# osmosis-diffusion/osmosis-diffusion-code

Hardware: AMD Instinct MI355X
Metric: denoise-steps/sec (256x256 RGBD, 1000-step DDPM+guidance) (higher is better)
Workload: dtype f32 (f16x3 conv)

## Files before the change

osmosis_diffusion_code_amd/_lib.py:

```python
import ctypes as C
import os
import threading
from typing import List, Optional, Tuple

import torch

_HERE = os.path.dirname(os.path.abspath(__file__))
LIB_PATH = os.environ.get("OSM_LIB") or os.path.join(_HERE, "libosmosis_hip.so")

c_float_p = C.c_void_p


class OsmosisHipError(RuntimeError):
    pass


class ConvDesc(C.Structure):
    _fields_ = [("x", C.c_void_p), ("w", C.c_void_p), ("bias", C.c_void_p), ("res", C.c_void_p),
                ("y", C.c_void_p), ("splitk_ws", C.c_void_p),
                ("B", C.c_int), ("H", C.c_int), ("W", C.c_int), ("Cin", C.c_int), ("Cout", C.c_int),
                ("ksize", C.c_int), ("splitk", C.c_int), ("accumulate", C.c_int),
                ("ldx", C.c_longlong), ("ldy", C.c_longlong), ("ldr", C.c_longlong), ("wfmt", C.c_int),
                ("gn_table", C.c_void_p), ("gn_silu", C.c_int),
                ("colsum", C.c_void_p), ("stat_mode", C.c_int), ("stat_silu", C.c_int), ("stat_x", C.c_void_p),
# ... 183 lines not shown
                                _P, _P, _I, _I, _P, _P],
}
EXPORTS_PHYSGROUP = sorted(_SIGS_PHYSGROUP)
_D = C.c_double
_SIGS_BLIND = {
    "osm_psf_tap_grad": [_P, _P, _P, _P, _I, _I, _I, _I, _I, _LL, _LL, _I, _I, _P, _P],
    "osm_psf_tap_step": [_P, _P, _P, _I, _I, _I, _LL, _D, _D, _P],
    "osm_ps_blind_optimize": [_P, _P, _P, _P, _P, _P, _I, _I, _I, _I, _I, _I, _I, _P, _P, _P, _P, _P, _P, _I, _D, _D, _P],
}
EXPORTS_BLIND = sorted(_SIGS_BLIND)
_SIGS_DEPTHPRIOR = {
    "osm_depth_nblk": [_I],
    "osm_depth_reduce": [C.POINTER(DepthDesc), _P, _P, _P, _P, _P],
    "osm_depth_fit": [C.POINTER(DepthDesc), _P, _P, _P, _P],
    "osm_depth_grad": [C.POINTER(DepthDesc), _P, _P, _P, _P, _P, _P],
    "osm_depth_loss_grad": [C.POINTER(DepthDesc), _P, _P, _P, _P, _P, _P, _P, _P],
}
EXPORTS_DEPTHPRIOR = sorted(_SIGS_DEPTHPRIOR)
_SIGS_SOLVER = {
    "osm_solver_update_c": [_P, _P, _P, _P, _P, _P, _P, _P, _P, _F, _P, _P, _P, _I, _I, _I, _P],
    "osm_solver_update_rng_c": [_P, _P, _P, _P, _P, _P, _P, _P, _F, _P, _P, _P, _I, _I, _I, C.c_ulonglong, _P, _I, _I, _I, _I, _P],
}
EXPORTS_SOLVER = sorted(_SIGS_SOLVER)

_lib = None
_lock = threading.Lock()


def load():
    global _lib
    if _lib is not None:
        return _lib
    with _lock:
        if _lib is None:
            if not os.path.exists(LIB_PATH):
                raise OsmosisHipError(
                    f"{LIB_PATH} is missing: build it with `python -c 'import __graft_entry__ as g; g.build()'` "
                    "or `make -C osmosis_diffusion_code_amd/csrc` (hipcc, --offload-arch=gfx950). "
                    "There is no CPU fallback for the product path.")
            lib = C.CDLL(LIB_PATH)
            for name, argtypes in list(_SIGS.items()) + list(_SIGS_LINOP.items()) + list(_SIGS_PSF.items()) + list(_SIGS_PHYSLIN.items()) + \
                    list(_SIGS_PHYSGROUP.items()) + list(_SIGS_BLIND.items()) + list(_SIGS_DEPTHPRIOR.items()) + list(_SIGS_SOLVER.items()):
                fn = getattr(lib, name)
                fn.argtypes = argtypes
                fn.restype = C.c_int
            lib.osm_packed_weight_elems.argtypes = [_I, _I, _I, _I, _I]
            lib.osm_packed_weight_elems.restype = C.c_longlong
            lib.osm_winograd_weight_elems.argtypes = [_I, _I, _I, _I]
            lib.osm_winograd_weight_elems.restype = C.c_longlong
            lib.osm_quantile_abs_ws_bytes.argtypes = [_LL]
            lib.osm_quantile_abs_ws_bytes.restype = C.c_longlong
            lib.osm_last_error.argtypes = []
            lib.osm_last_error.restype = C.c_char_p
            _lib = lib
    return _lib


class Recorder:

    def __init__(self):
        self.calls: List[Tuple] = []
        self.keep: List = []

    def __enter__(self):
        _state.recorders.append(self)
        return self

    def __exit__(self, *exc):
        _state.recorders.pop()
        return False

    @staticmethod
    def suspended():
        class _Suspend:
# ... 99 lines not shown
```

osmosis_diffusion_code_amd/csrc/guidance.hip:

```cpp
#include "osm_common.h"
#include "depth_conv.h"
#include "../../include/osmosis_linop.h"
#include "../../include/osmosis_psf.h"
#include "../../include/osmosis_physlin.h"
#include "../../include/osmosis_physgroup.h"
#include "../../include/osmosis_solver.h"

namespace {

constexpr int PPB = 1024;
constexpr int NRED = 16;

template <bool MASKED> struct PixMask { float wm[3]; };
template <> struct PixMask<false> {};

template <bool MASKED>
struct Pix : PixMask<MASKED> {
  float rgb[3], D, y[3];
  float d, dd, w;
  float Ea[3], Eb[3], J[3], r[3];
};

template <bool MASKED, bool FMA_I = false, bool MODEL_ONLY = false>
__device__ __forceinline__ void eval_pixel(const osm_phys_desc& ds, const float* __restrict__ x0,
                                           const float* __restrict__ y, const float* __restrict__ mask,
                                           const float* __restrict__ phi, int b, int p, Pix<MASKED>& q) {
  const long long base = (long long)b * 4 * ds.HW + p;
  float m[3] = {1.f, 1.f, 1.f};
#pragma unroll
  for (int c = 0; c < 3; ++c) {
    q.rgb[c] = x0[base + (long long)c * ds.HW];
    if constexpr (!MODEL_ONLY) q.y[c] = y[(long long)b * 3 * ds.HW + (long long)c * ds.HW + p];
    if constexpr (MASKED) m[c] = mask[(long long)b * 3 * ds.HW + (long long)c * ds.HW + p];
  }
  q.D = x0[base + 3LL * ds.HW];
  if (ds.kind == 3) {
    q.d = 0.f; q.dd = 0.f; q.w = 1.f;
#pragma unroll
    for (int c = 0; c < 3; ++c) {
      q.Ea[c] = q.Eb[c] = 1.f;
      q.J[c] = 0.5f * (q.rgb[c] + 1.0f);
      q.r[c] = q.y[c] - q.rgb[c];
      if constexpr (MASKED) { q.wm[c] = m[c]; q.r[c] *= m[c]; }
    }
    return;
  }
  q.d = conv_depth(q.D, ds.depth_type, ds.dval, q.dd);
  float wdd;
  q.w = ds.weight_type == 1 ? conv_depth(q.D, ds.wdepth_type, ds.wval, wdd) : 1.0f;
  const float* ph = phi + b * 9;
#pragma unroll
  for (int c = 0; c < 3; ++c) {
    const float pa = ds.kind == 2 ? ph[0] : ph[c];
    const float pb = ds.kind == 0 ? ph[3 + c] : pa;
    const float pinf = ph[6 + c];
    q.Ea[c] = expf(-pa * q.d);
    q.Eb[c] = expf(-pb * q.d);
    q.J[c] = 0.5f * (q.rgb[c] + 1.0f);
    float I;
    if constexpr (FMA_I) {
      I = fmaf(q.J[c], q.Ea[c], pinf * (1.0f - q.Eb[c]));
    } else {
      I = q.J[c] * q.Ea[c] + pinf * (1.0f - q.Eb[c]);
    }
    if constexpr (MODEL_ONLY) {
      q.r[c] = I;
    } else if constexpr (MASKED) {
      q.wm[c] = q.w * m[c];
      q.r[c] = (q.y[c] - (2.0f * I - 1.0f)) * q.wm[c];
    } else {
      q.r[c] = (q.y[c] - (2.0f * I - 1.0f)) * q.w;
    }
  }
}

template <bool MASKED, bool LIN>
__global__ __launch_bounds__(256) void phys_reduce_kernel(osm_phys_desc ds, const float* __restrict__ x0,
                                                           const float* __restrict__ y,
                                                           const float* __restrict__ mask,
                                                           const float* __restrict__ phi, const float* __restrict__ v,
                                                           float* __restrict__ part, int nblk) {
  static_assert(!(MASKED && LIN), "the composed route's mask acts on the measurement's grid (phys_resid_kernel)");
  __shared__ float red[4][NRED];
  const int b = blockIdx.y, blk = blockIdx.x;
  float s[NRED];
#pragma unroll
  for (int k = 0; k < NRED; ++k) s[k] = 0.f;
  const int pend = min(ds.HW, (blk + 1) * PPB);
  const float* ph = phi + b * 9;
  for (int p = blk * PPB + threadIdx.x; p < pend; p += 256) {
    Pix<MASKED> q;
    eval_pixel<MASKED, false, LIN>(ds, x0, y, mask, phi, b, p, q);
#pragma unroll
    for (int c = 0; c < 3; ++c) {
      const float pinf = ph[6 + c];
      float k2;
      if constexpr (LIN) {
        k2 = v[((long long)b * 3 + c) * ds.HW + p];
      } else {
        float wc = q.w;
        if constexpr (MASKED) wc = q.wm[c];
        k2 = -2.0f * wc * q.r[c];
        s[0] += q.r[c] * q.r[c];
      }
      s[1 + c] += k2 * (-q.d * q.J[c] * q.Ea[c]);
      s[4 + c] += k2 * (pinf * q.d * q.Eb[c]);
      s[7 + c] += k2 * (1.0f - q.Eb[c]);
      s[10 + c] += q.rgb[c];
      const float e = fmaxf(fabsf(q.rgb[c]) - 0.7f, 0.0f);
      s[13] += e * e;
    }
  }
  const int lane = threadIdx.x & 63, wv = threadIdx.x >> 6;
#pragma unroll
  for (int k = 0; k < NRED; ++k) {
    const float t = osm::wave_sum(s[k]);
    if (lane == 0) red[wv][k] = t;
  }
  __syncthreads();
  if (threadIdx.x < NRED) {
    const int k = threadIdx.x;
    part[((long long)b * nblk + blk) * NRED + k] = (red[0][k] + red[1][k]) + (red[2][k] + red[3][k]);
  }
}

__device__ __forceinline__ float sgn(float v) { return (v > 0.f) ? 1.f : ((v < 0.f) ? -1.f : 0.f); }

__device__ __forceinline__ int phys_param_lr(const osm_phys_desc& ds, float* lr) {
  for (int i = 0; i < 9; ++i) lr[i] = 0.f;
  int live;
  if (ds.kind == 0) {
    for (int c = 0; c < 3; ++c) { lr[c] = ds.eta[0]; lr[3 + c] = ds.eta[1]; }
    live = 0x3f;
  } else if (ds.kind == 1) {
    for (int c = 0; c < 3; ++c) lr[c] = ds.eta[0];
    live = 0x7;
  } else {
    lr[0] = ds.eta[0];
    live = 0x1;
  }
  for (int c = 0; c < 3; ++c) lr[6 + c] = ds.eta[2];
  return live | 0x1c0;
}

__device__ __forceinline__ void phys_param_grad(const osm_phys_desc& ds, const double* tot, double gscale, double* dg) {
  for (int i = 0; i < 9; ++i) dg[i] = 0.0;
  if (ds.kind == 0) {
    for (int c = 0; c < 3; ++c) {
// ... 93 lines not shown
}

template <bool LIN> struct FinLin { const float* part_r; int nblk_r, hw; };
template <> struct FinLin<false> {};

template <bool LIN>
__device__ __forceinline__ void fin_walk(const float* __restrict__ part, float* __restrict__ red, int nblk, const FinLin<LIN>& lin,
                                         int b, int lane, double* tot) {
  static_assert(NRED * 4 == 64, "one wave covers the components");
  const int comp = lane >> 2, sub = lane & 3;
  double a = 0.0;
#pragma unroll 4
  for (int k = sub; k < nblk; k += 4) a += (double)part[((long long)b * nblk + k) * NRED + comp];
  if constexpr (LIN) {
    if (comp == 0) {
      a = 0.0;
      for (int k = sub; k < lin.nblk_r; k += 4) a += (double)lin.part_r[(long long)b * lin.nblk_r + k];
    }
  }
  a += __shfl_xor(a, 1, 64);
  a += __shfl_xor(a, 2, 64);
  if (sub == 0) {
    tot[comp] = a;
    red[b * NRED + comp] = (float)a;
  }
}

template <bool LIN>
__device__ __forceinline__ bool fin_member(const osm_phys_desc& ds, const double* tot, const FinLin<LIN>& lin, int zero_guard, int b,
                                           float* __restrict__ loss_out, int do_update, double* dg) {
  double n = 3.0 * (double)ds.HW;
  if constexpr (LIN) n = 3.0 * (double)lin.hw;
  double L, gscale;
  bool live = true;
  if (ds.loss_type == 0) {
    L = sqrt(tot[0]);
    gscale = 1.0 / L;
    if (zero_guard && tot[0] == 0.0) { gscale = 0.0; live = false; }
  } else {
    L = tot[0] / n;
    gscale = 2.0 / n;
  }
  if (loss_out) loss_out[b] = (float)L;
  if (do_update) phys_param_grad(ds, tot, gscale, dg);
  return live;
}

__device__ __forceinline__ void fin_step(const osm_phys_desc& ds, const double* dg, double omega, float* ph, float* st) {
  float g[9], lr[9];
  const int live = phys_param_lr(ds, lr);
  for (int i = 0; i < 9; ++i) g[i] = (float)(dg[i] * omega);
  phys_opt_step(ds, g, lr, live, ph, st);
}

template <bool LIN>
__global__ void phys_finalize_kernel(osm_phys_desc ds, const float* __restrict__ part, float* __restrict__ red,
                                     float* __restrict__ phi, int do_update, float* __restrict__ loss_out,
                                     float* __restrict__ opt_state, int nblk, int zero_guard, const FinLin<LIN> lin) {
  __shared__ double tot[NRED];
  const int b = blockIdx.x;
  fin_walk(part, red, nblk, lin, b, threadIdx.x, tot);
  __syncthreads();
  if (threadIdx.x == 0) {
    double dg[9];
    if (fin_member(ds, tot, lin, zero_guard, b, loss_out, do_update, dg) && do_update)
      fin_step(ds, dg, 1.0, phi + b * 9, opt_state ? opt_state + b * 20 : nullptr);
  }
}

struct GroupOff { int G, reduce_mean, off[OSM_MAX_GROUPS + 1]; };
constexpr int GWAVES = 4;

template <bool LIN>
__global__ __launch_bounds__(64 * GWAVES) void phys_finalize_group_kernel(osm_phys_desc ds, const float* __restrict__ part,
                                                                          float* __restrict__ red, float* phi, int do_update,
                                                                          float* __restrict__ loss_out, float* opt_state, int nblk,
                                                                          int zero_guard, const GroupOff go, const FinLin<LIN> lin) {
  __shared__ double tot[GWAVES][NRED];
  __shared__ double dsh[GWAVES][9];
  __shared__ int live_sh[GWAVES];
  __shared__ float row[9 + 20];
  __shared__ int stepped;
  const int b0 = go.off[blockIdx.x], n = go.off[blockIdx.x + 1] - b0;
  const int wv = threadIdx.x >> 6, lane = threadIdx.x & 63;
  double acc[9];
  int any = 0;
  for (int r0 = 0; r0 < n; r0 += GWAVES) {
    const int m = r0 + wv;
    if (m < n) fin_walk(part, red, nblk, lin, b0 + m, lane, tot[wv]);
    __syncthreads();
// ... 9 lines not shown
  }
  if (threadIdx.x == 0) {
    stepped = 0;
    if (do_update && any) {
      float* ph = phi + b0 * 9;
      float* st = opt_state ? opt_state + b0 * 20 : nullptr;
      fin_step(ds, acc, go.reduce_mean ? 1.0 / (double)n : 1.0, ph, st);
      for (int i = 0; i < 9; ++i) row[i] = ph[i];
      for (int i = 0; i < 20; ++i) row[9 + i] = st ? st[i] : 0.f;
      stepped = 1;
    }
  }
  __syncthreads();
  if (stepped) {
    for (int idx = threadIdx.x; idx < (n - 1) * 29; idx += 64 * GWAVES) {
      const int b = b0 + 1 + idx / 29, k = idx % 29;
      if (k < 9) phi[b * 9 + k] = row[k];
      else if (opt_state) opt_state[b * 20 + (k - 9)] = row[k];
    }
  }
}

template <bool MASKED, bool LIN>
__global__ __launch_bounds__(256) void phys_grad_kernel(osm_phys_desc ds, const float* __restrict__ x0,
                                                         const float* __restrict__ y,
                                                         const float* __restrict__ mask,
                                                         const float* __restrict__ phi, const float* __restrict__ v,
                                                         const float* __restrict__ red, float* __restrict__ g, int hw,
                                                         int zero_guard) {
  static_assert(!(MASKED && LIN), "the composed route's mask acts on the measurement's grid (phys_resid_kernel)");
  const int b = blockIdx.y;
  const int p = blockIdx.x * 256 + threadIdx.x;
  if (p >= ds.HW) return;
  Pix<MASKED> q;
  eval_pixel<MASKED, MASKED, LIN>(ds, x0, y, mask, phi, b, p, q);
  const float* rd = red + b * NRED;
  const float n = 3.0f * (float)ds.HW;
  float gscale = ds.loss_type == 0 ? 1.0f / sqrtf(rd[0]) : 2.0f / (LIN ? 3.0f * (float)hw : n);
  if ((MASKED || (LIN && zero_guard)) && ds.loss_type == 0 && rd[0] == 0.f) gscale = 0.f;
  const float* ph = phi + b * 9;
  float gD = 0.f;
  const long long base = (long long)b * 4 * ds.HW + p;
  if constexpr (!LIN) {
    if (ds.kind == 3) {
#pragma unroll
      for (int c = 0; c < 3; ++c) {
        if constexpr (MASKED) g[base + (long long)c * ds.HW] = -(q.wm[c] * (q.r[c] * gscale));
        else g[base + (long long)c * ds.HW] = -(q.r[c] * gscale);
      }
      g[base + 3LL * ds.HW] = 0.f;
      return;
    }
  }
#pragma unroll
  for (int c = 0; c < 3; ++c) {
    const float pa = ds.kind == 2 ? ph[0] : ph[c];
    const float pb = ds.kind == 0 ? ph[3 + c] : pa;
    const float pinf = ph[6 + c];
    float dLdI;
    if constexpr (LIN) {
      dLdI = v[((long long)b * 3 + c) * ds.HW + p] * gscale;
    } else {
      float wc = q.w;
      if constexpr (MASKED) wc = q.wm[c];
      dLdI = -2.0f * wc * (q.r[c] * gscale);
    }
    float grgb = dLdI * 0.5f * q.Ea[c];
    if (ds.gamma_avrg != 0.f) grgb += ds.gamma_avrg * sgn(rd[10 + c]) / (float)ds.HW;
    if (ds.gamma_val != 0.f) {
      const float e = fmaxf(fabsf(q.rgb[c]) - 0.7f, 0.0f);
      grgb += ds.gamma_val * 2.0f * e * sgn(q.rgb[c]) / n;
    }
    g[base + (long long)c * ds.HW] = grgb;
    gD += dLdI * (-pa * q.J[c] * q.Ea[c] + pinf * pb * q.Eb[c]) * q.dd;
  }
  g[base + 3LL * ds.HW] = gD;
}


__global__ __launch_bounds__(256) void phys_forward_kernel(osm_phys_desc ds, const float* __restrict__ x0,
                                                            const float* __restrict__ phi, float* __restrict__ F, int P) {
  const int b = blockIdx.y;
  const int p = blockIdx.x * 256 + threadIdx.x;
  if (p >= ds.HW) return;
  Pix<false> q;
  eval_pixel<false, true, true>(ds, x0, nullptr, nullptr, phi, b, p, q);
  const long long base = (long long)b * P * ds.HW + p;
#pragma unroll
  for (int c = 0; c < 3; ++c) F[base + (long long)c * ds.HW] = q.r[c];
  if (P == 4) F[base + 3LL * ds.HW] = q.w;
}

__global__ __launch_bounds__(256) void phys_resid_kernel(const float* __restrict__ AF, const float* __restrict__ y,
                                                          const float* __restrict__ mask, float* __restrict__ u,
                                                          float* __restrict__ part_r, int P, int hw, int nblk) {
  __shared__ float red[4];
  const int b = blockIdx.y, blk = blockIdx.x;
  float s = 0.f;
  const int pend = min(hw, (blk + 1) * PPB);
  for (int p = blk * PPB + threadIdx.x; p < pend; p += 256) {
    const float wt = P == 4 ? AF[((long long)b * P + 3) * hw + p] : 1.0f;
#pragma unroll
    for (int c = 0; c < 3; ++c) {
      const long long e = ((long long)b * 3 + c) * hw + p;
      const float wm = mask ? wt * mask[e] : wt;
      const float r = (y[e] - (2.0f * AF[((long long)b * P + c) * hw + p] - 1.0f)) * wm;
      u[e] = -2.0f * wm * r;
      s += r * r;
    }
// ... 361 lines not shown
}

inline int grid_for(long long total) {
  long long b = (total + 255) / 256;
  if (b > 2048) b = 2048;
  return (int)(b < 1 ? 1 : b);
}

int check_desc(const osm_phys_desc* d, const char* who) {
  OSM_REQUIRE(d, "%s: null descriptor", who);
  OSM_REQUIRE(d->kind >= 0 && d->kind <= 3, "%s: unknown operator kind %d", who, d->kind);
  OSM_REQUIRE(d->kind != 3 || (d->loss_type == 0 && d->weight_type == 0 && d->gamma_avrg == 0.f && d->gamma_val == 0.f),
              "%s: the identity operator (kind 3) is the plain norm loss: no weight, no auxiliary losses", who);
  OSM_REQUIRE(d->depth_type >= 0 && d->depth_type <= 2, "%s: unknown depth_type %d", who, d->depth_type);
  OSM_REQUIRE(d->loss_type == 0 || d->loss_type == 1, "%s: unknown loss_type %d", who, d->loss_type);
  OSM_REQUIRE(d->B > 0 && d->HW > 0, "%s: bad shape", who);
  return OSM_OK;
}

}

extern "C" int osm_phys_nblk(int HW) { return (HW + PPB - 1) / PPB; }

namespace {
int check_lin_desc(const osm_phys_desc* d, const char* who) {
  int rc = check_desc(d, who);
  if (rc) return rc;
  OSM_REQUIRE(d->kind != 3, "%s: the identity operator (kind 3) has no image-formation model to compose with", who);
  return OSM_OK;
}

int check_phi_step(const char* who, const osm_phys_desc* d, int do_update, const float* opt_state) {
  OSM_REQUIRE(d->optimizer >= 0 && d->optimizer <= 8, "%s: optimizer must be 0 (sgd / GD) .. 8 (see osm_phys_desc)", who);
  OSM_REQUIRE(!(d->optimizer != 0 && do_update) || opt_state, "%s: a stateful optimizer needs opt_state [B][20]", who);
  OSM_REQUIRE(!(d->kind == 3 && do_update), "%s: the identity operator (kind 3) has no parameters to step", who);
  return OSM_OK;
}

struct LinArgs { int hw; const float* v; const float* part_r; };

int phys_reduce_launch(const char* who, const osm_phys_desc* d, const float* x0, const float* y, const float* mask, const float* phi,
                       float* part, void* stream, const LinArgs* la = nullptr) {
  int rc = la ? check_lin_desc(d, who) : check_desc(d, who);
  if (rc) return rc;
  OSM_REQUIRE(x0 && phi && part && (la ? la->v != nullptr : y != nullptr), "%s: null pointer", who);
  const int nblk = osm_phys_nblk(d->HW);
// ... 157 lines not shown

extern "C" int osm_phys_reduce_lin(const osm_phys_desc* d, const float* x0, const float* phi, const float* v, float* part,
                                   void* stream) {
  const LinArgs la{0, v, nullptr};
  return phys_reduce_launch("osm_phys_reduce_lin", d, x0, nullptr, nullptr, phi, part, stream, &la);
}

extern "C" int osm_phys_finalize_lin(const osm_phys_desc* d, int hw, const float* part, const float* part_r, float* red, float* phi,
                                     int do_update, float* loss_out, float* opt_state, int masked, void* stream) {
  const LinArgs la{hw, nullptr, part_r};
  return phys_finalize_launch("osm_phys_finalize_lin", d, part, red, phi, do_update, loss_out, opt_state, masked != 0, stream, nullptr,
                              &la);
}

extern "C" int osm_phys_grad_lin(const osm_phys_desc* d, int hw, const float* x0, const float* phi, const float* v, const float* red,
                                 float* g, int masked, void* stream) {
  const LinArgs la{hw, v, nullptr};
  return phys_grad_launch("osm_phys_grad_lin", d, x0, nullptr, nullptr, phi, red, g, stream, &la, masked != 0);
}

namespace {
struct LinWs { const osm_lin_desc* lin; float *F, *AF, *u, *v, *part_r; };

int phys_optimize_launch(const char* who, const osm_phys_desc* d, const float* x0, const float* y, const float* mask, float* phi,
                         float* part, float* red, float* loss_out, float* g, int n_inner, int freeze_phi, float* opt_state,
                         void* stream, const GroupOff* go = nullptr, const LinWs* lw = nullptr) {
  int rc = lw ? check_lin_desc(d, who) : check_desc(d, who);
  if (rc) return rc;
  if (lw && (rc = check_lin(d, lw->lin, who))) return rc;
  OSM_REQUIRE(x0 && y && phi && part && red && loss_out && g && (!lw || (lw->F && lw->AF && lw->u && lw->v && lw->part_r)),
              "%s: null pointer", who);
  OSM_REQUIRE(n_inner >= 1, "%s: n_inner must be >= 1", who);
  OSM_REQUIRE(!(freeze_phi && n_inner != 1), "%s: freeze_phi goes with n_inner = 1", who);
  if ((rc = check_phi_step(who, d, !freeze_phi, opt_state))) return rc;
  OSM_REQUIRE(!lw || (long long)d->B * 4 <= 65535, "%s: batch %d is too large for one launch of the operator", who, d->B);
  const int zg = mask != nullptr, hw = lw ? lw->lin->h * lw->lin->w : 0, P = lin_planes(d);
  const LinArgs la_{hw, lw ? lw->v : nullptr, lw ? lw->part_r : nullptr}, *la = lw ? &la_ : nullptr;
  for (int it = 0; it < n_inner; ++it) {
    if (lw) {
      if ((rc = osm_phys_forward(d, x0, phi, lw->F, stream))) return rc;
      if ((rc = lin_apply(lw->lin, lw->F, lw->AF, d->B, P, 0, stream))) return rc;
      if ((rc = osm_phys_resid(d, hw, lw->AF, y, mask, lw->u, lw->part_r, stream))) return rc;
      if ((rc = lin_apply(lw->lin, lw->u, lw->v, d->B, 3, 1, stream))) return rc;
    }
    if ((rc = phys_reduce_launch(who, d, x0, y, mask, phi, part, stream, la))) return rc;
    if (it < n_inner - 1) {
      if ((rc = phys_finalize_launch(who, d, part, red, phi, 1, loss_out, opt_state, zg, stream, go, la))) return rc;
      continue;
    }
    if ((rc = phys_finalize_launch(who, d, part, red, phi, 0, loss_out, nullptr, zg, stream, go, la))) return rc;
    if ((rc = phys_grad_launch(who, d, x0, y, mask, phi, red, g, stream, la, zg))) return rc;
    if (!freeze_phi && (rc = phys_finalize_launch(who, d, part, red, phi, 1, nullptr, opt_state, zg, stream, go, la))) return rc;
  }
  return OSM_OK;
}
}

extern "C" int osm_phys_optimize(const osm_phys_desc* d, const float* x0, const float* y, float* phi, float* part, float* red,
// ... 504 lines not shown
```

osmosis_diffusion_code_amd/guided_diffusion/condition_methods.py:

```python
from abc import ABC, abstractmethod
from functools import partial

import os
import torch

from .. import ops
from .._lib import PhysDesc
from ..osmosis_utils import losses as losseso
from ..osmosis_utils import utils as utilso

__CONDITIONING_METHOD__ = {}


def register_conditioning_method(name: str):
    def wrapper(cls):
        if __CONDITIONING_METHOD__.get(name, None):
            raise NameError(f"Name {name} is already registered!")
        __CONDITIONING_METHOD__[name] = cls
        return cls
    return wrapper


def get_conditioning_method(name: str, operator, noiser, **kwargs):
    if __CONDITIONING_METHOD__.get(name, None) is None:
# ... 340 lines not shown
            raise NotImplementedError
        d = PhysDesc()
        op.fill_desc(d)
        if self.loss_weight in (None, "none"):
            d.weight_type, d.wdepth_type = 0, 0
        elif self.loss_weight == "depth":
            fn, value = utilso.parse_weight_function(self.weight_function)
            code, vals = utilso.depth_code_and_values(fn if fn != "none" else None, value)
            d.weight_type, d.wdepth_type = 1, code
            for i in range(3):
                d.wval[i] = vals[i]
        else:
            raise NotImplementedError
        d.loss_type = 0 if self.loss_function == "norm" else 1
        coefs = self.aux_loss.kernel_coefficients() if self.aux_loss is not None else {"gamma_avrg": 0.0, "gamma_val": 0.0}
        d.gamma_avrg, d.gamma_val = coefs["gamma_avrg"], coefs["gamma_val"]
        d.B, d.HW = B, HW
        from .measurements import OPTIMIZER_CODES
        d.optimizer = OPTIMIZER_CODES.get(getattr(op, "optimizer", "") or "", 0)
        nblk = ops.phys_nblk(HW)
        if d.optimizer != 0 and (self._opt is None or self._opt.shape[0] != op.phi.shape[0] or self._opt.device != op.phi.device):
            self._opt = torch.zeros(op.phi.shape[0], 20, device=device, dtype=torch.float32)
        st = {"key": key, "desc": d,
              "part": torch.empty(B * nblk * 16, device=device, dtype=torch.float32),
              "red": torch.zeros(B * 16, device=device, dtype=torch.float32),
              "loss": torch.zeros(B, device=device, dtype=torch.float32),
              "g": torch.empty(B, 4, HW, device=device, dtype=torch.float32)}
        if grid is not None:
            lin = ops.lin_desc(self._degradation(), grid[0], grid[1], device)
            hw, P = lin.h * lin.w, ops.phys_lin_planes(d)
            f32 = dict(device=device, dtype=torch.float32)
            st.update(lin=lin, hw=hw, F=torch.empty(B, P, HW, **f32), AF=torch.empty(B, P, hw, **f32), u=torch.empty(B, 3, hw, **f32),
                      v=torch.empty(B, 3, HW, **f32), part_r=torch.empty(B * ops.phys_nblk(hw), **f32))
        while len(self._states) >= 4:
            self._states.pop(next(iter(self._states)))
        self._states[st["key"]] = st
        self._state = st
        return st

    def _group(self, phi):
        sizes = getattr(self.operator, "group_sizes", None)
        if sizes is None:
            return None
        full = self.operator.phi
        if phi.data_ptr() != full.data_ptr() or phi.shape[0] != full.shape[0]:
            raise ValueError(f"phi_groups: a water group spans chunks -- the data term got {phi.shape[0]} phi rows of the operator's "
                             f"{full.shape[0]}; a grouped batch takes ONE call over all its images")
# ... 256 lines not shown
        s = self.scale.to(torch.float32)
        if s.numel() not in (1, channels):
            raise ValueError(f"scale must have 1 or {channels} entries")
        return (s.repeat(channels) if s.numel() == 1 else s).to(device).contiguous()

    def loss_grad_x0(self, x0, y, g_out=None, loss_out=None, mask=None):
        from .measurements import GRID_OPERATORS
        if self._blind() is not None:
            return self._loss_grad_x0_blind(x0, y, g_out, loss_out, mask)
        if isinstance(self.operator, GRID_OPERATORS):
            return self._loss_grad_x0_separable(x0, y, g_out, loss_out, mask)
        B, C, HW = x0.shape[0], x0.shape[1], x0.shape[2] * x0.shape[3]
        if y.shape[0] != B or y.shape[1] != 3 or C not in (3, 4):
            raise ValueError("expected x0 [B,4,H,W] or [B,3,H,W] and measurement [B,3,H,W]")
        key = (B, HW, str(x0.device)) if C == 4 else (B, HW, str(x0.device), C)
        st = self._states.get(key)
        if st is None:
            f32 = dict(device=x0.device, dtype=torch.float32)
            if C == 4:
                d = PhysDesc()
                d.kind, d.depth_type, d.weight_type, d.wdepth_type, d.loss_type, d.optimizer = 3, 0, 0, 0, 0, 0
                d.gamma_avrg = d.gamma_val = 0.0
                d.B, d.HW = B, HW
                st = {"desc": d, "part": torch.empty(B * ops.phys_nblk(HW) * 16, **f32), "red": torch.zeros(B * 16, **f32),
                      "loss": torch.zeros(B, **f32), "g": torch.empty(B, 4, HW, **f32), "phi": torch.zeros(B, 9, **f32)}
            else:
                st = {"part": torch.empty(B * ops.phys_nblk(HW), **f32), "loss": torch.zeros(B, **f32),
                      "g": torch.empty(B, C, HW, **f32)}
            while len(self._states) >= 4:
                self._states.pop(next(iter(self._states)))
            self._states[key] = st
        g = g_out if g_out is not None else st["g"]
        loss = loss_out if loss_out is not None else st["loss"]
        if mask is None:
            mask = self.measurement_mask(B, HW, x0.device)
        if mask is not None and C == 4:
            ops.phys_optimize_m(st["desc"], x0.contiguous(), y.contiguous(), mask, st["phi"], st["part"], st["red"], loss, g, 1, True)
        elif mask is not None:
            ops.ps_loss_grad_mc(x0.contiguous(), y.contiguous(), mask, st["part"], loss, g, B, C, HW)
        elif C == 4:
            ops.phys_optimize(st["desc"], x0.contiguous(), y.contiguous(), st["phi"], st["part"], st["red"], loss, g, 1, True)
        else:
            ops.ps_loss_grad_c(x0.contiguous(), y.contiguous(), st["part"], loss, g, B, C, HW)
        return g.view(x0.shape), loss

    def _loss_grad_x0_separable(self, x0, y, g_out=None, loss_out=None, mask=None):
        from .measurements import PSFOperator
# ... 91 lines not shown
```

osmosis_diffusion_code_amd/ops.py:

```python
import ctypes as C
from dataclasses import dataclass
from typing import Optional

import torch

from . import _lib
from ._lib import AttnDesc, ConvDesc, DepthDesc, GemmDesc, GroupDesc, LinDesc, PhysDesc, ReconDesc, call, current_stream_ptr, ptr, ptr_f64, query


@dataclass
class Mat:
    t: torch.Tensor
    rows: int
    cols: int
    ld: int

    @staticmethod
    def of(t: torch.Tensor) -> "Mat":
        if t.dim() != 2 or (t.shape[1] > 1 and t.stride(1) != 1):
            raise _lib.OsmosisHipError("Mat.of needs a 2-D view with unit column stride")
        return Mat(t, t.shape[0], t.shape[1], t.stride(0) if t.shape[0] > 1 else max(t.stride(0), t.shape[1]))

    @property
    def p(self) -> int:
# ... 328 lines not shown
def quantile_workspace(n: int, device) -> torch.Tensor:
    return torch.empty(-(-quantile_ws_bytes(n) // 4), device=device, dtype=torch.int32)


def quantile_abs(x, s, q, idx, ws):
    assert x.is_contiguous() and q.numel() >= 1 and idx.numel() >= 2 and idx.dtype == torch.int32
    call("osm_quantile_abs", ptr(x), x.numel(), float(s), ptr(q), ptr(idx), ptr(ws), _s(), keep=(x, q, idx, ws))


def posterior_dynthr(model_out, x, coef, x0, mean, logvar, x0_raw, q, idx, ws, B, HW, mean_kind=0, var_kind=0, s=0.98):
    call("osm_posterior_dynthr", ptr(model_out), ptr(x), ptr(coef), int(mean_kind), int(var_kind), float(s), ptr(x0_raw), ptr(x0),
         ptr(mean), ptr(logvar), ptr(q), ptr(idx), ptr(ws), B, HW, _s(), keep=(model_out, x, coef, x0_raw, x0, mean, logvar, q, idx, ws))


def dynthr_bwd(g, x_raw, q, idx, ws, s=0.98):
    assert g.numel() == x_raw.numel() and g.is_contiguous() and x_raw.is_contiguous()
    call("osm_dynthr_bwd", ptr(g), ptr(x_raw), ptr(q), ptr(idx), float(s), g.numel(), ptr(ws), _s(), keep=(g, x_raw, q, idx, ws))


def phys_nblk(HW):
    return query("osm_phys_nblk", HW)


def phys_reduce(desc: PhysDesc, x0, y, phi, part):
    call("osm_phys_reduce", C.byref(desc), ptr(x0), ptr(y), ptr(phi), ptr(part), _s(), keep=(desc, x0, y, phi, part))


def phys_finalize(desc: PhysDesc, part, red, phi, do_update, loss_out, opt_state=None):
    call("osm_phys_finalize", C.byref(desc), ptr(part), ptr(red), ptr(phi), int(do_update), ptr(loss_out), ptr(opt_state), _s(),
         keep=(part, red, phi, loss_out, opt_state))


def phys_grad(desc: PhysDesc, x0, y, phi, red, g):
    call("osm_phys_grad", C.byref(desc), ptr(x0), ptr(y), ptr(phi), ptr(red), ptr(g), _s(),
         keep=(desc, x0, y, phi, red, g))


def phys_optimize(desc: PhysDesc, x0, y, phi, part, red, loss_out, g, n_inner: int, freeze_phi: bool, opt_state=None):
    call("osm_phys_optimize", C.byref(desc), ptr(x0), ptr(y), ptr(phi), ptr(part), ptr(red), ptr(loss_out), ptr(g), int(n_inner),
         int(bool(freeze_phi)), ptr(opt_state), _s(), keep=(desc, x0, y, phi, part, red, loss_out, g, opt_state))


def _check_mask(mask, y):
    if mask is not None and (mask.numel() != y.numel() or not mask.is_contiguous() or mask.dtype != torch.float32):
        raise ValueError(f"mask must be contiguous fp32 with the measurement's {y.numel()} elements ([B,3,HW]), "
                         f"got {tuple(mask.shape)} {mask.dtype}")


def phys_reduce_m(desc: PhysDesc, x0, y, mask, phi, part):
    _check_mask(mask, y)
    call("osm_phys_reduce_m", C.byref(desc), ptr(x0), ptr(y), ptr(mask), ptr(phi), ptr(part), _s(), keep=(desc, x0, y, mask, phi, part))


def phys_finalize_m(desc: PhysDesc, part, red, phi, do_update, loss_out, opt_state=None, masked=True):
    call("osm_phys_finalize_m", C.byref(desc), ptr(part), ptr(red), ptr(phi), int(do_update), ptr(loss_out), ptr(opt_state),
         int(bool(masked)), _s(), keep=(part, red, phi, loss_out, opt_state))


def phys_grad_m(desc: PhysDesc, x0, y, mask, phi, red, g):
    _check_mask(mask, y)
    call("osm_phys_grad_m", C.byref(desc), ptr(x0), ptr(y), ptr(mask), ptr(phi), ptr(red), ptr(g), _s(),
         keep=(desc, x0, y, mask, phi, red, g))


def phys_optimize_m(desc: PhysDesc, x0, y, mask, phi, part, red, loss_out, g, n_inner: int, freeze_phi: bool, opt_state=None):
    _check_mask(mask, y)
    call("osm_phys_optimize_m", C.byref(desc), ptr(x0), ptr(y), ptr(mask), ptr(phi), ptr(part), ptr(red), ptr(loss_out), ptr(g),
         int(n_inner), int(bool(freeze_phi)), ptr(opt_state), _s(), keep=(desc, x0, y, mask, phi, part, red, loss_out, g, opt_state))


def exposure_mask(y, mask_out, B, HW, low, high, soft=0.0, per_pixel=False):
    assert y.numel() == B * 3 * HW and mask_out.numel() == B * 3 * HW and y.is_contiguous() and mask_out.is_contiguous()
    call("osm_exposure_mask", ptr(y), float(low), float(high), float(soft), int(bool(per_pixel)), ptr(mask_out), B, HW, _s(),
         keep=(y, mask_out))


def posterior_bwd(g, coef, d_out, B, HW):
    call("osm_posterior_bwd", ptr(g), ptr(coef), ptr(d_out), B, HW, _s(), keep=(g, coef, d_out))


def guide_update(mean, logvar, g, dx_unet, noise, coef, scale4, clip, x_next, grad_out, B, HW):
    call("osm_guide_update", ptr(mean), ptr(logvar), ptr(g), ptr(dx_unet), ptr(noise), ptr(coef), ptr(scale4),
         float(clip), ptr(x_next), ptr(grad_out), B, HW, _s(),
         keep=(mean, logvar, g, dx_unet, noise, coef, scale4, x_next, grad_out))


def guide_update_rng(mean, logvar, g, dx_unet, coef, scale4, clip, x_next, grad_out, noise_out, B, HW, seed, step, step_offset=0,
                     img0=0, img_stride=1):
    call("osm_guide_update_rng", ptr(mean), ptr(logvar), ptr(g), ptr(dx_unet), ptr(coef), ptr(scale4), float(clip), ptr(x_next),
# ... 441 lines not shown
```

osmosis_diffusion_code_amd/torch_ops.py:

```python
import itertools
import weakref
from typing import List, Optional, Tuple

import torch

from . import ops
from ._lib import OsmosisHipError, PhysDesc

_ENGINES = weakref.WeakValueDictionary()
_next_handle = itertools.count(1)


def engine_handle(eng) -> int:
    h = getattr(eng, "_osm_handle", None)
    if h is None:
        h = eng._osm_handle = next(_next_handle)
    _ENGINES[h] = eng
    return h


def _engine(handle: int):
    eng = _ENGINES.get(int(handle))
    if eng is None:
        raise OsmosisHipError(f"osmosis:: operator called with a stale engine handle ({handle}): the engine was released")
# ... 254 lines not shown
def _mask_rows(name, mask, y):
    if mask.dim() != 4 or mask.shape[0] != y.shape[0] or mask.shape[1] not in (1, 3) or mask.shape[2:] != y.shape[2:]:
        raise OsmosisHipError(f"{name}: expected mask [B,3,H,W] or [B,1,H,W] on the measurement's grid")
    return mask.expand(y.shape).contiguous()


def _phys_loss_grad_impl(name, x0, y, mask, phi, icfg, fcfg, n_inner, freeze_phi, grp=None):
    B, HW = _chw(x0)
    if len(icfg) != len(PHYS_ICFG) or len(fcfg) != len(PHYS_FCFG):
        raise OsmosisHipError(f"{name}: icfg / fcfg must come from torch_ops.phys_config(desc)")
    d = PhysDesc()
    for k, v in zip(PHYS_ICFG, icfg):
        setattr(d, k, int(v))
    if d.optimizer != 0:
        raise OsmosisHipError(f"{name} is functional: optimizer state (adam, ...) lives with the conditioning method")
    if d.kind == 3 and not freeze_phi:
        raise OsmosisHipError(f"{name}: the identity operator (kind 3) has no parameters: pass freeze_phi=True")
    for i in range(3):
        d.dval[i], d.wval[i], d.eta[i] = fcfg[i], fcfg[3 + i], fcfg[8 + i]
    d.gamma_avrg, d.gamma_val = fcfg[6], fcfg[7]
    d.B, d.HW = B, HW
    dev = x0.device
    phi_new = phi.detach().clone().contiguous()
    part = torch.empty(B * ops.phys_nblk(HW) * 16, device=dev, dtype=torch.float32)
    red = torch.zeros(B * 16, device=dev, dtype=torch.float32)
    loss = torch.zeros(B, device=dev, dtype=torch.float32)
    g = torch.empty_like(x0)
    if grp is not None:
        ops.phys_optimize_g(d, grp, x0, y.contiguous(), None if mask is None else _mask_rows(name, mask, y), phi_new, part, red, loss, g,
                            1 if freeze_phi else n_inner, freeze_phi)
    elif mask is None:
        ops.phys_optimize(d, x0, y.contiguous(), phi_new, part, red, loss, g, 1 if freeze_phi else n_inner, freeze_phi)
    else:
        ops.phys_optimize_m(d, x0, y.contiguous(), _mask_rows(name, mask, y), phi_new, part, red, loss, g,
                            1 if freeze_phi else n_inner, freeze_phi)
    return loss, g, phi_new


@phys_loss_grad.register_fake
def _phys_loss_grad_fake(x0, y, phi, icfg, fcfg, n_inner, freeze_phi):
    return x0.new_empty((x0.shape[0],)), torch.empty_like(x0), torch.empty_like(phi)


@torch.library.custom_op("osmosis::phys_loss_grad_m", mutates_args=(), device_types="cuda")
def phys_loss_grad_m(x0: torch.Tensor, y: torch.Tensor, mask: torch.Tensor, phi: torch.Tensor, icfg: List[int], fcfg: List[float],
                     n_inner: int, freeze_phi: bool) -> Tuple[torch.Tensor, torch.Tensor, torch.Tensor]:
    return _phys_loss_grad_impl("osmosis::phys_loss_grad_m", x0, y, mask, phi, icfg, fcfg, n_inner, freeze_phi)
# ... 446 lines not shown
```

Before: 56.07.

## Fuse phys parameter finalize/step into next reduce and grad kernels

Replaces the per-inner-iteration reduce, finalize and step launch sequence of phys_optimize with one fused step kernel per iteration. Each block redundantly walks the previous partial sums, applies the optimizer step to a shared-memory copy of phi, then runs the next reduction. A final grad kernel also folds in the last finalize. Ping-pong buffers for partials, phi and optimizer state live in an enlarged workspace. This cuts kernel launches and serialization in the guidance step, at the cost of duplicated finalize work in every block and a larger workspace.

```diff
diff --git a/include/osmosis_physstep.h b/include/osmosis_physstep.h
--- /dev/null
+++ b/include/osmosis_physstep.h
@@ -0,0 +1,13 @@
+#ifndef OSMOSIS_PHYSSTEP_H
+#define OSMOSIS_PHYSSTEP_H
+
+#ifdef __cplusplus
+extern "C" {
+#endif
+
+long long osm_phys_optimize_ws(int B, int HW);
+
+#ifdef __cplusplus
+}
+#endif
+#endif
diff --git a/osmosis_diffusion_code_amd/_lib.py b/osmosis_diffusion_code_amd/_lib.py
--- a/osmosis_diffusion_code_amd/_lib.py
+++ b/osmosis_diffusion_code_amd/_lib.py
@@ -229,6 +229,10 @@
     "osm_solver_update_rng_c": [_P, _P, _P, _P, _P, _P, _P, _P, _F, _P, _P, _P, _I, _I, _I, C.c_ulonglong, _P, _I, _I, _I, _I, _P],
 }
 EXPORTS_SOLVER = sorted(_SIGS_SOLVER)
+_SIGS_PHYSSTEP = {
+    "osm_phys_optimize_ws": [_I, _I],
+}
+EXPORTS_PHYSSTEP = sorted(_SIGS_PHYSSTEP)
 
 _lib = None
 _lock = threading.Lock()
@@ -257,6 +261,8 @@
             lib.osm_winograd_weight_elems.restype = C.c_longlong
             lib.osm_quantile_abs_ws_bytes.argtypes = [_LL]
             lib.osm_quantile_abs_ws_bytes.restype = C.c_longlong
+            lib.osm_phys_optimize_ws.argtypes = _SIGS_PHYSSTEP["osm_phys_optimize_ws"]
+            lib.osm_phys_optimize_ws.restype = C.c_longlong
             lib.osm_last_error.argtypes = []
             lib.osm_last_error.restype = C.c_char_p
             _lib = lib
diff --git a/osmosis_diffusion_code_amd/csrc/guidance.hip b/osmosis_diffusion_code_amd/csrc/guidance.hip
--- a/osmosis_diffusion_code_amd/csrc/guidance.hip
+++ b/osmosis_diffusion_code_amd/csrc/guidance.hip
@@ -5,6 +5,7 @@
 #include "../../include/osmosis_physlin.h"
 #include "../../include/osmosis_physgroup.h"
 #include "../../include/osmosis_solver.h"
+#include "../../include/osmosis_physstep.h"
 
 namespace {
 
@@ -24,7 +25,7 @@
 template <bool MASKED, bool FMA_I = false, bool MODEL_ONLY = false>
 __device__ __forceinline__ void eval_pixel(const osm_phys_desc& ds, const float* __restrict__ x0,
                                            const float* __restrict__ y, const float* __restrict__ mask,
-                                           const float* __restrict__ phi, int b, int p, Pix<MASKED>& q) {
+                                           const float* __restrict__ ph, int b, int p, Pix<MASKED>& q) {
   const long long base = (long long)b * 4 * ds.HW + p;
   float m[3] = {1.f, 1.f, 1.f};
 #pragma unroll
@@ -48,7 +49,6 @@
   q.d = conv_depth(q.D, ds.depth_type, ds.dval, q.dd);
   float wdd;
   q.w = ds.weight_type == 1 ? conv_depth(q.D, ds.wdepth_type, ds.wval, wdd) : 1.0f;
-  const float* ph = phi + b * 9;
 #pragma unroll
   for (int c = 0; c < 3; ++c) {
     const float pa = ds.kind == 2 ? ph[0] : ph[c];
@@ -75,11 +75,9 @@
 }
 
 template <bool MASKED, bool LIN>
-__global__ __launch_bounds__(256) void phys_reduce_kernel(osm_phys_desc ds, const float* __restrict__ x0,
-                                                           const float* __restrict__ y,
-                                                           const float* __restrict__ mask,
-                                                           const float* __restrict__ phi, const float* __restrict__ v,
-                                                           float* __restrict__ part, int nblk) {
+__device__ __forceinline__ void reduce_block(const osm_phys_desc& ds, const float* __restrict__ x0, const float* __restrict__ y,
+                                             const float* __restrict__ mask, const float* __restrict__ ph,
+                                             const float* __restrict__ v, float* __restrict__ part, int nblk) {
   static_assert(!(MASKED && LIN), "the composed route's mask acts on the measurement's grid (phys_resid_kernel)");
   __shared__ float red[4][NRED];
   const int b = blockIdx.y, blk = blockIdx.x;
@@ -87,10 +85,9 @@
 #pragma unroll
   for (int k = 0; k < NRED; ++k) s[k] = 0.f;
   const int pend = min(ds.HW, (blk + 1) * PPB);
-  const float* ph = phi + b * 9;
   for (int p = blk * PPB + threadIdx.x; p < pend; p += 256) {
     Pix<MASKED> q;
-    eval_pixel<MASKED, false, LIN>(ds, x0, y, mask, phi, b, p, q);
+    eval_pixel<MASKED, false, LIN>(ds, x0, y, mask, ph, b, p, q);
 #pragma unroll
     for (int c = 0; c < 3; ++c) {
       const float pinf = ph[6 + c];
@@ -124,6 +121,22 @@
   }
 }
 
+template <bool MASKED, bool LIN>
+__global__ __launch_bounds__(256) void phys_reduce_kernel(osm_phys_desc ds, const float* __restrict__ x0,
+                                                           const float* __restrict__ y,
+                                                           const float* __restrict__ mask,
+                                                           const float* __restrict__ phi, const float* __restrict__ v,
+                                                           float* __restrict__ part, int nblk) {
+  if constexpr (LIN) {
+    reduce_block<MASKED, LIN>(ds, x0, y, mask, phi + blockIdx.y * 9, v, part, nblk);
+  } else {
+    float ph[9];
+#pragma unroll
+    for (int i = 0; i < 9; ++i) ph[i] = phi[blockIdx.y * 9 + i];
+    reduce_block<MASKED, LIN>(ds, x0, y, mask, ph, v, part, nblk);
+  }
+}
+
 __device__ __forceinline__ float sgn(float v) { return (v > 0.f) ? 1.f : ((v < 0.f) ? -1.f : 0.f); }
 
 __device__ __forceinline__ int phys_param_lr(const osm_phys_desc& ds, float* lr) {
@@ -263,7 +276,7 @@
   a += __shfl_xor(a, 2, 64);
   if (sub == 0) {
     tot[comp] = a;
-    red[b * NRED + comp] = (float)a;
+    if (red) red[b * NRED + comp] = (float)a;
   }
 }
 
@@ -291,7 +304,13 @@
   float g[9], lr[9];
   const int live = phys_param_lr(ds, lr);
   for (int i = 0; i < 9; ++i) g[i] = (float)(dg[i] * omega);
-  phys_opt_step(ds, g, lr, live, ph, st);
+  float p[9], s[20];
+  for (int i = 0; i < 9; ++i) p[i] = ph[i];
+  for (int i = 0; i < 20; ++i) s[i] = st ? st[i] : 0.f;
+  phys_opt_step(ds, g, lr, live, p, s);
+  for (int i = 0; i < 9; ++i) ph[i] = p[i];
+  if (st)
+    for (int i = 0; i < 20; ++i) st[i] = s[i];
 }
 
 template <bool LIN>
@@ -307,6 +326,39 @@
     if (fin_member(ds, tot, lin, zero_guard, b, loss_out, do_update, dg) && do_update)
       fin_step(ds, dg, 1.0, phi + b * 9, opt_state ? opt_state + b * 20 : nullptr);
   }
+}
+
+template <bool MASKED>
+__global__ __launch_bounds__(256) void phys_step_kernel(osm_phys_desc ds, const float* __restrict__ x0, const float* __restrict__ y,
+                                                         const float* __restrict__ mask, const float* __restrict__ part_prev,
+                                                         float* __restrict__ part, const float* __restrict__ phi_src,
+                                                         const float* __restrict__ st_src, float* __restrict__ phi_dst,
+                                                         float* __restrict__ st_dst, float* __restrict__ red,
+                                                         float* __restrict__ loss_out, int nblk, int prev, int zero_guard) {
+  __shared__ double tot[NRED];
+  __shared__ float row[9 + 20];
+  const int b = blockIdx.y, t = threadIdx.x;
+  const bool writer = blockIdx.x == 0;
+  if (t < 64) {
+    if (t < 9) row[t] = phi_src[b * 9 + t];
+    else if (t < 29 && st_src) row[t] = st_src[b * 20 + (t - 9)];
+    if (prev) fin_walk(part_prev, writer ? red : nullptr, nblk, FinLin<false>{}, b, t, tot);
+  }
+  __syncthreads();
+  if (t == 0 && prev) {
+    double dg[9];
+    if (fin_member(ds, tot, FinLin<false>{}, zero_guard, b, writer ? loss_out : nullptr, 1, dg))
+      fin_step(ds, dg, 1.0, row, st_src ? row + 9 : nullptr);
+  }
+  __syncthreads();
+  if (writer && phi_dst) {
+    if (t < 9) phi_dst[b * 9 + t] = row[t];
+    else if (t < 29 && st_dst) st_dst[b * 20 + (t - 9)] = row[t];
+  }
+  float ph[9];
+#pragma unroll
+  for (int i = 0; i < 9; ++i) ph[i] = row[i];
+  reduce_block<MASKED, false>(ds, x0, y, mask, ph, nullptr, part, nblk);
 }
 
 struct GroupOff { int G, reduce_mean, off[OSM_MAX_GROUPS + 1]; };
@@ -362,23 +414,15 @@
 }
 
 template <bool MASKED, bool LIN>
-__global__ __launch_bounds__(256) void phys_grad_kernel(osm_phys_desc ds, const float* __restrict__ x0,
-                                                         const float* __restrict__ y,
-                                                         const float* __restrict__ mask,
-                                                         const float* __restrict__ phi, const float* __restrict__ v,
-                                                         const float* __restrict__ red, float* __restrict__ g, int hw,
-                                                         int zero_guard) {
+__device__ __forceinline__ void grad_pixel(const osm_phys_desc& ds, const float* __restrict__ x0, const float* __restrict__ y,
+                                           const float* __restrict__ mask, const float* __restrict__ ph, const float* __restrict__ v,
+                                           const float* __restrict__ rd, float* __restrict__ g, int hw, int zero_guard, int b, int p) {
   static_assert(!(MASKED && LIN), "the composed route's mask acts on the measurement's grid (phys_resid_kernel)");
-  const int b = blockIdx.y;
-  const int p = blockIdx.x * 256 + threadIdx.x;
-  if (p >= ds.HW) return;
   Pix<MASKED> q;
-  eval_pixel<MASKED, MASKED, LIN>(ds, x0, y, mask, phi, b, p, q);
-  const float* rd = red + b * NRED;
+  eval_pixel<MASKED, MASKED, LIN>(ds, x0, y, mask, ph, b, p, q);
   const float n = 3.0f * (float)ds.HW;
   float gscale = ds.loss_type == 0 ? 1.0f / sqrtf(rd[0]) : 2.0f / (LIN ? 3.0f * (float)hw : n);
   if ((MASKED || (LIN && zero_guard)) && ds.loss_type == 0 && rd[0] == 0.f) gscale = 0.f;
-  const float* ph = phi + b * 9;
   float gD = 0.f;
   const long long base = (long long)b * 4 * ds.HW + p;
   if constexpr (!LIN) {
@@ -417,6 +461,50 @@
   g[base + 3LL * ds.HW] = gD;
 }
 
+template <bool MASKED, bool LIN>
+__global__ __launch_bounds__(256) void phys_grad_kernel(osm_phys_desc ds, const float* __restrict__ x0,
+                                                         const float* __restrict__ y,
+                                                         const float* __restrict__ mask,
+                                                         const float* __restrict__ phi, const float* __restrict__ v,
+                                                         const float* __restrict__ red, float* __restrict__ g, int hw,
+                                                         int zero_guard) {
+  const int b = blockIdx.y;
+  const int p = blockIdx.x * 256 + threadIdx.x;
+  if (p >= ds.HW) return;
+  grad_pixel<MASKED, LIN>(ds, x0, y, mask, phi + b * 9, v, red + b * NRED, g, hw, zero_guard, b, p);
+}
+
+template <bool MASKED>
+__global__ __launch_bounds__(256) void phys_grad_step_kernel(osm_phys_desc ds, const float* __restrict__ x0,
+                                                              const float* __restrict__ y, const float* __restrict__ mask,
+                                                              const float* __restrict__ part_prev, const float* __restrict__ phi_src,
+                                                              const float* __restrict__ st_src, float* __restrict__ phi_dst,
+                                                              float* __restrict__ st_dst, float* __restrict__ red,
+                                                              float* __restrict__ loss_out, float* __restrict__ g, int nblk,
+                                                              int do_update, int zero_guard) {
+  __shared__ double tot[NRED];
+  const int b = blockIdx.y, t = threadIdx.x;
+  const bool writer = blockIdx.x == 0;
+  if (t < 64) fin_walk(part_prev, writer ? red : nullptr, nblk, FinLin<false>{}, b, t, tot);
+  __syncthreads();
+  if (writer && t == 0) {
+    double dg[9];
+    const bool live = fin_member(ds, tot, FinLin<false>{}, zero_guard, b, loss_out, do_update, dg);
+    if (do_update) {
+      for (int i = 0; i < 9; ++i) phi_dst[b * 9 + i] = phi_src[b * 9 + i];
+      if (st_dst)
+        for (int i = 0; i < 20; ++i) st_dst[b * 20 + i] = st_src[b * 20 + i];
+      if (live) fin_step(ds, dg, 1.0, phi_dst + b * 9, st_dst ? st_dst + b * 20 : nullptr);
+    }
+  }
+  const int p = blockIdx.x * 256 + t;
+  if (p >= ds.HW) return;
+  float rd[NRED];
+#pragma unroll
+  for (int k = 0; k < NRED; ++k) rd[k] = (float)tot[k];
+  grad_pixel<MASKED, false>(ds, x0, y, mask, phi_src + b * 9, nullptr, rd, g, 0, 0, b, p);
+}
+
 
 __global__ __launch_bounds__(256) void phys_forward_kernel(osm_phys_desc ds, const float* __restrict__ x0,
                                                             const float* __restrict__ phi, float* __restrict__ F, int P) {
@@ -424,7 +512,7 @@
   const int p = blockIdx.x * 256 + threadIdx.x;
   if (p >= ds.HW) return;
   Pix<false> q;
-  eval_pixel<false, true, true>(ds, x0, nullptr, nullptr, phi, b, p, q);
+  eval_pixel<false, true, true>(ds, x0, nullptr, nullptr, phi + b * 9, b, p, q);
   const long long base = (long long)b * P * ds.HW + p;
 #pragma unroll
   for (int c = 0; c < 3; ++c) F[base + (long long)c * ds.HW] = q.r[c];
@@ -832,6 +920,11 @@
 
 extern "C" int osm_phys_nblk(int HW) { return (HW + PPB - 1) / PPB; }
 
+extern "C" long long osm_phys_optimize_ws(int B, int HW) {
+  if (B <= 0 || HW <= 0) return -1;
+  return (long long)B * (2LL * osm_phys_nblk(HW) * NRED + 9 + 20);
+}
+
 namespace {
 int check_lin_desc(const osm_phys_desc* d, const char* who) {
   int rc = check_desc(d, who);
@@ -1035,6 +1128,53 @@
 namespace {
 struct LinWs { const osm_lin_desc* lin; float *F, *AF, *u, *v, *part_r; };
 
+
+struct StepBufs {
+  float *part[2], *phi[2], *st[2];
+};
+
+int phys_steps_launch(const osm_phys_desc* d, const float* x0, const float* y, const float* mask, float* phi, float* part, float* red,
+                      float* loss_out, float* g, int n_inner, int freeze_phi, float* opt_state, hipStream_t st) {
+  const int nblk = osm_phys_nblk(d->HW), zg = mask != nullptr, nv = freeze_phi ? 0 : n_inner;
+  const long long np = (long long)d->B * nblk * NRED;
+  StepBufs bf;
+  bf.part[0] = part;
+  bf.part[1] = part + np;
+  bf.phi[0] = phi;
+  bf.phi[1] = part + 2 * np;
+  bf.st[0] = opt_state;
+  bf.st[1] = opt_state ? part + 2 * np + (long long)d->B * 9 : nullptr;
+  auto side = [nv](int j) { return (nv - j) & 1; };
+  const dim3 grid(nblk, d->B), block(256);
+  for (int k = 0; k < n_inner; ++k) {
+    const int src = k == 0 ? 0 : side(k - 1), dst = side(k);
+    const float* pprev = k ? bf.part[(k - 1) & 1] : nullptr;
+    float* pdst = (k == 0 && dst == 0) ? nullptr : bf.phi[dst];
+    if (mask)
+      hipLaunchKernelGGL(phys_step_kernel<true>, grid, block, 0, st, *d, x0, y, mask, pprev, bf.part[k & 1], bf.phi[src], bf.st[src], pdst,
+                         bf.st[dst], red, loss_out, nblk, k != 0, zg);
+    else
+      hipLaunchKernelGGL(phys_step_kernel<false>, grid, block, 0, st, *d, x0, y, nullptr, pprev, bf.part[k & 1], bf.phi[src], bf.st[src],
+                         pdst, bf.st[dst], red, loss_out, nblk, k != 0, zg);
+    int rc = osm::check_launch("phys_step_kernel");
+    if (rc) return rc;
+  }
+  const int src = freeze_phi ? 0 : side(n_inner - 1), dst = side(n_inner);
+  const dim3 ggrid((d->HW + 255) / 256, d->B);
+  if (mask)
+    hipLaunchKernelGGL(phys_grad_step_kernel<true>, ggrid, block, 0, st, *d, x0, y, mask, bf.part[(n_inner - 1) & 1], bf.phi[src],
+                       bf.st[src], bf.phi[dst], bf.st[dst], red, loss_out, g, nblk, !freeze_phi, zg);
+  else
+    hipLaunchKernelGGL(phys_grad_step_kernel<false>, ggrid, block, 0, st, *d, x0, y, nullptr, bf.part[(n_inner - 1) & 1], bf.phi[src],
+                       bf.st[src], bf.phi[dst], bf.st[dst], red, loss_out, g, nblk, !freeze_phi, zg);
+  return osm::check_launch("phys_grad_step_kernel");
+}
+
+bool unfused_phys_steps() {
+  const char* e = std::getenv("OSM_PHYS_STEP_FUSED");
+  return e && e[0] == '0';
+}
+
 int phys_optimize_launch(const char* who, const osm_phys_desc* d, const float* x0, const float* y, const float* mask, float* phi,
                          float* part, float* red, float* loss_out, float* g, int n_inner, int freeze_phi, float* opt_state,
                          void* stream, const GroupOff* go = nullptr, const LinWs* lw = nullptr) {
@@ -1047,6 +1187,8 @@
   OSM_REQUIRE(!(freeze_phi && n_inner != 1), "%s: freeze_phi goes with n_inner = 1", who);
   if ((rc = check_phi_step(who, d, !freeze_phi, opt_state))) return rc;
   OSM_REQUIRE(!lw || (long long)d->B * 4 <= 65535, "%s: batch %d is too large for one launch of the operator", who, d->B);
+  if (!go && !lw && !unfused_phys_steps())
+    return phys_steps_launch(d, x0, y, mask, phi, part, red, loss_out, g, n_inner, freeze_phi, opt_state, (hipStream_t)stream);
   const int zg = mask != nullptr, hw = lw ? lw->lin->h * lw->lin->w : 0, P = lin_planes(d);
   const LinArgs la_{hw, lw ? lw->v : nullptr, lw ? lw->part_r : nullptr}, *la = lw ? &la_ : nullptr;
   for (int it = 0; it < n_inner; ++it) {
diff --git a/osmosis_diffusion_code_amd/guided_diffusion/condition_methods.py b/osmosis_diffusion_code_amd/guided_diffusion/condition_methods.py
--- a/osmosis_diffusion_code_amd/guided_diffusion/condition_methods.py
+++ b/osmosis_diffusion_code_amd/guided_diffusion/condition_methods.py
@@ -386,7 +386,7 @@
         if d.optimizer != 0 and (self._opt is None or self._opt.shape[0] != op.phi.shape[0] or self._opt.device != op.phi.device):
             self._opt = torch.zeros(op.phi.shape[0], 20, device=device, dtype=torch.float32)
         st = {"key": key, "desc": d,
-              "part": torch.empty(B * nblk * 16, device=device, dtype=torch.float32),
+              "part": torch.empty(ops.phys_optimize_ws(B, HW), device=device, dtype=torch.float32),
               "red": torch.zeros(B * 16, device=device, dtype=torch.float32),
               "loss": torch.zeros(B, device=device, dtype=torch.float32),
               "g": torch.empty(B, 4, HW, device=device, dtype=torch.float32)}
@@ -689,7 +689,7 @@
                 d.kind, d.depth_type, d.weight_type, d.wdepth_type, d.loss_type, d.optimizer = 3, 0, 0, 0, 0, 0
                 d.gamma_avrg = d.gamma_val = 0.0
                 d.B, d.HW = B, HW
-                st = {"desc": d, "part": torch.empty(B * ops.phys_nblk(HW) * 16, **f32), "red": torch.zeros(B * 16, **f32),
+                st = {"desc": d, "part": torch.empty(ops.phys_optimize_ws(B, HW), **f32), "red": torch.zeros(B * 16, **f32),
                       "loss": torch.zeros(B, **f32), "g": torch.empty(B, 4, HW, **f32), "phi": torch.zeros(B, 9, **f32)}
             else:
                 st = {"part": torch.empty(B * ops.phys_nblk(HW), **f32), "loss": torch.zeros(B, **f32),
diff --git a/osmosis_diffusion_code_amd/ops.py b/osmosis_diffusion_code_amd/ops.py
--- a/osmosis_diffusion_code_amd/ops.py
+++ b/osmosis_diffusion_code_amd/ops.py
@@ -374,6 +374,19 @@
     return query("osm_phys_nblk", HW)
 
 
+def phys_optimize_ws(B, HW):
+    n = query("osm_phys_optimize_ws", int(B), int(HW))
+    if n < 0:
+        raise _lib.OsmosisHipError(f"phys_optimize workspace of a batch of {B} images of {HW} pixels")
+    return int(n)
+
+
+def _check_step_ws(desc, part):
+    need = phys_optimize_ws(desc.B, desc.HW)
+    if part.numel() < need or part.dtype != torch.float32 or not part.is_contiguous():
+        raise ValueError(f"part must be contiguous fp32 with phys_optimize_ws(B, HW) = {need} elements, got {part.numel()} {part.dtype}")
+
+
 def phys_reduce(desc: PhysDesc, x0, y, phi, part):
     call("osm_phys_reduce", C.byref(desc), ptr(x0), ptr(y), ptr(phi), ptr(part), _s(), keep=(desc, x0, y, phi, part))
 
@@ -389,6 +402,7 @@
 
 
 def phys_optimize(desc: PhysDesc, x0, y, phi, part, red, loss_out, g, n_inner: int, freeze_phi: bool, opt_state=None):
+    _check_step_ws(desc, part)
     call("osm_phys_optimize", C.byref(desc), ptr(x0), ptr(y), ptr(phi), ptr(part), ptr(red), ptr(loss_out), ptr(g), int(n_inner),
          int(bool(freeze_phi)), ptr(opt_state), _s(), keep=(desc, x0, y, phi, part, red, loss_out, g, opt_state))
 
@@ -417,6 +431,7 @@
 
 def phys_optimize_m(desc: PhysDesc, x0, y, mask, phi, part, red, loss_out, g, n_inner: int, freeze_phi: bool, opt_state=None):
     _check_mask(mask, y)
+    _check_step_ws(desc, part)
     call("osm_phys_optimize_m", C.byref(desc), ptr(x0), ptr(y), ptr(mask), ptr(phi), ptr(part), ptr(red), ptr(loss_out), ptr(g),
          int(n_inner), int(bool(freeze_phi)), ptr(opt_state), _s(), keep=(desc, x0, y, mask, phi, part, red, loss_out, g, opt_state))
 
diff --git a/osmosis_diffusion_code_amd/torch_ops.py b/osmosis_diffusion_code_amd/torch_ops.py
--- a/osmosis_diffusion_code_amd/torch_ops.py
+++ b/osmosis_diffusion_code_amd/torch_ops.py
@@ -300,7 +300,7 @@
     d.B, d.HW = B, HW
     dev = x0.device
     phi_new = phi.detach().clone().contiguous()
-    part = torch.empty(B * ops.phys_nblk(HW) * 16, device=dev, dtype=torch.float32)
+    part = torch.empty(ops.phys_optimize_ws(B, HW), device=dev, dtype=torch.float32)
     red = torch.zeros(B * 16, device=dev, dtype=torch.float32)
     loss = torch.zeros(B, device=dev, dtype=torch.float32)
     g = torch.empty_like(x0)
```

Result: no change. 56.24 (median of 6 runs) (+0.3%).
